# PythonOptimizers/pysparse

Hardware: AMD Instinct MI355X
Metric: CSR SpMV GB/s (7-pt Poisson, % of 8 TB/s HBM peak) + PCG iters/s (higher is better)
Workload: dtype f64

## Files before the change

### pysparse_amd/csrc/psp_csr_abi.h

```cpp

__global__ __launch_bounds__(256) void csr_validate_kernel(int nnz, int ncols, const int *__restrict__ col,
                                                           unsigned long long *bad) {
  for (long k = (long)blockIdx.x * 256 + threadIdx.x; k < nnz; k += (long)gridDim.x * 256) {
    const int c = col[k];
    if (c < 0 || c >= ncols) atomicMin(bad, (unsigned long long)k);
  }
}

extern "C" {

int psp_csr_create(int nrows, int ncols, int nnz, const int *ind_host, const int *col_host,
                   const double *val_host, psp_csr_t **out) {
  if (psp::cpu_mode()) return psp::cpu::csr_create(nrows, ncols, nnz, ind_host, col_host, val_host, out);
  if (!out || !ind_host || (nnz > 0 && (!col_host || !val_host)))
    return fail(PSP_EINVAL, "psp_csr_create: NULL argument");
  if (nrows < 0 || ncols < 0 || nnz < 0) return fail(PSP_EINVAL, "psp_csr_create: negative size");
  if (ind_host[0] != 0 || ind_host[nrows] != nnz)
    return fail(PSP_EINVAL, "psp_csr_create: ind[0] must be 0 and ind[nrows] == nnz");
  for (int i = 0; i < nrows; ++i)
    if (ind_host[i + 1] < ind_host[i])
      return fail(PSP_EINVAL, "psp_csr_create: ind not monotone at row %d", i);
  const bool check_on_device = nnz >= (1 << 22);
  if (!check_on_device)
    for (int k = 0; k < nnz; ++k)
// ... 39 lines not shown
  const long nnz = poisson_prefix(row_hi, nx, ny, nz) - poisson_prefix(row_lo, nx, ny, nz);
  if (nloc > 0x7fffffffL || nnz > 0x7fffffffL || ncols_local < 0)
    return fail(PSP_EINVAL, "psp_csr_poisson: local part exceeds 32-bit indices");
  const long reach = nz > 0 ? (long)nx * ny : nx;
  long cmin = (row_lo - reach > 0 ? row_lo - reach : 0) - col_shift;
  long cmax = (row_hi - 1 + reach < n - 1 ? row_hi - 1 + reach : n - 1) - col_shift;
  if (nloc > 0 && (cmin < 0 || cmax >= ncols_local))
    return fail(PSP_EINVAL, "psp_csr_poisson: col_shift/ncols_local do not cover the halo");
  psp_csr *A;
  PSP_TRY(alloc_csr((int)nloc, ncols_local, nnz, &A));
  int grid = (int)std::min<long>((nloc + 1 + 255) / 256, 8192);
  hipLaunchKernelGGL(poisson_csr_kernel, dim3(grid), dim3(256), 0, stream(), nx, ny, nz,
                     (long)row_lo, (long)row_hi, (long)col_shift, A->ind, A->col, A->val);
  PSP_LAUNCH_CHECK();
  PSP_TRY(finalize_csr(A));
  *out = A;
  return PSP_OK;
}

int psp_csr_poisson(int nx, int ny, int nz, psp_csr_t **out) {
  if (psp::cpu_mode()) return out ? psp::cpu::csr_poisson(nx, ny, nz, out) : fail(PSP_EINVAL, "psp_csr_poisson: NULL argument");
  const long n = (long)nx * ny * (nz > 0 ? nz : 1);
  if (n > 0x7fffffffL) return fail(PSP_EINVAL, "psp_csr_poisson: n exceeds 32-bit indices");
  return psp_csr_poisson_slab(nx, ny, nz, 0, n, 0, (int)n, out);
}

int psp_csr_poisson_big_slab(int nx, int ny, int nz, int64_t row_lo, int64_t row_hi, int64_t col_shift,
                             int ncols_local, psp_csr_t **out) {
  if (!out || nx < 2 || ny < 2 || nz < 0 || nz == 1)
    return fail(PSP_EINVAL, "psp_csr_poisson_big: grid dimensions must be >= 2 (nz = 0: 2-D)");
// ... 44 lines not shown
  hipError_t e1 = hipMalloc((void **)&ex->dia_val, sizeof(double) * nval);
  hipError_t e2 = hipMalloc((void **)&ex->dia_mask, sizeof(unsigned short) * (nblk * kDiaRows + 2));
  if (e1 != hipSuccess || e2 != hipSuccess) {
    (void)hipGetLastError();
    psp_csr_destroy(A);
    return fail(PSP_ENOMEM, "psp_csr_poisson_big: device allocation of %zu values failed", nval);
  }
  PSP_HIP(hipMemsetAsync(ex->dia_val, 0, sizeof(double) * nval, stream()));
  PSP_HIP(hipMemsetAsync(ex->dia_mask, 0, sizeof(unsigned short) * (nblk * kDiaRows + 2), stream()));
  hipLaunchKernelGGL(poisson_w4_kernel, dim3(65536), dim3(256), 0, stream(), nx, ny, nz, (long)row_lo, nloc, no,
                     ex->dia_val, ex->dia_mask);
  PSP_LAUNCH_CHECK();
  PSP_HIP(hipStreamSynchronize(stream()));
  ex->dia_no = no;
  ex->dia_state = 1;
  *out = A;
  return PSP_OK;
}

int psp_csr_poisson_big(int nx, int ny, int nz, psp_csr_t **out) {
  const long n = (long)nx * ny * (nz > 0 ? nz : 1);
  if (n > 0x7fffffffL - 256) return fail(PSP_EINVAL, "psp_csr_poisson_big: n exceeds 32-bit row indices");
  return psp_csr_poisson_big_slab(nx, ny, nz, 0, n, 0, (int)n, out);
}

int64_t psp_csr_nnz64(const psp_csr_t *A) {
  return A ? ((A->w4_only || A->nparts || A->multi) ? A->nnz64 : (int64_t)A->nnz) : 0;
}

static int create_part(int ncols, int64_t r0, int64_t r1, const int64_t *ind, const int *col, const double *val,
// ... 421 lines not shown
int psp_csr_setup_info(psp_csr_t *A, double *info4) {
  PSP_API_GUARD_H(A);
  if (!A || !info4) return fail(PSP_EINVAL, "psp_csr_setup_info: NULL argument");
  info4[0] = info4[1] = info4[2] = info4[3] = 0.0;
  if (A->host || A->multi || A->nparts) return PSP_OK;
  std::lock_guard<std::mutex> lk(g_extra_mu);
  auto it = g_extra.find(A);
  if (it == g_extra.end()) return PSP_OK;
  info4[0] = it->second.reorder_ms;
  info4[1] = (double)it->second.products;
  info4[2] = (double)reorder_after();
  info4[3] = (double)it->second.reorder_state;
  return PSP_OK;
}

int psp_csr_kernel_info(psp_csr_t *A, char *name, int name_cap, int *info) {
  PSP_API_GUARD_H(A);
  if (!A) return fail(PSP_EINVAL, "psp_csr_kernel_info: NULL handle");
  if (A->host) {
    if (name && name_cap > 0) snprintf(name, name_cap, "cpu loops (PSP_DEVICE=cpu)");
    if (info) info[0] = info[1] = info[2] = info[3] = 0;
    return PSP_OK;
  }
  if (A->multi) {
    char buf[160];
    psp::multi_describe(A->multi, buf, sizeof buf);
    if (name && name_cap > 0) snprintf(name, name_cap, "%s", buf);
    if (info) info[0] = info[1] = info[2] = info[3] = 0;
    return PSP_OK;
  }
  if (A->nparts) return psp_csr_kernel_info(A->parts[0], name, name_cap, info);
  Variant v = decode_variant(A->variant);
  if (A->w4_only) v.w4 = true;
  const char *k = "csr_spmv_stream";
  int vals[4] = {0, 0, 0, 0};
  bool w4 = false;
  if (v.w4 && A->sym_owner) {
    psp_sss *S = const_cast<psp_sss *>(A->sym_owner);
    PSP_TRY(ensure_sss_w4(S));
    if (S->w4_state == 1) {
      w4 = true;
      k = "sss_spmv_w4";
      vals[0] = S->w4_nol;
    }
  }
  if (!w4 && v.w4) {
    psp::CsrExtra *ex;
    PSP_TRY(ensure_w4(A, &ex));
    if (ex->dia_state == 1) {
      w4 = true;
      k = "csr_spmv_w4";
      vals[0] = ex->dia_no;
    }
  }
  if (!w4 && A->nrows > 0 && (v.wave || v.w1) && A->max_row_nnz <= v.tile / 2) {
    k = v.wave ? "csr_spmv_wave" : "csr_spmv_w1";
    if (v.w2) {
      ChunkTable *t;
      PSP_TRY(get_chunk_table(A, v.tile, &t));
      PSP_TRY(ensure_rowoff(A, t));
      if (t->np != 0) {
        k = "csr_spmv_w2";
        if (v.w3) {
          PSP_TRY(ensure_w3(A, t));
          vals[1] = t->max_blocks;
          {
            psp::CsrExtra *exs = nullptr;
// ... 379 lines not shown
```

### pysparse_amd/csrc/psp_csr_kernels.h

```cpp

constexpr int kBlock = 256;


__global__ void build_chunk_table(int nrows, const int *__restrict__ ind, int target, int nchunks,
                                  int2 *__restrict__ tab) {
  int c = blockIdx.x * blockDim.x + threadIdx.x;
  if (c > nchunks) return;
  int r;
  if (c == nchunks) {
    r = nrows;
  } else {
    long want = (long)c * target;
    int lo = 0, hi = nrows;
    while (lo < hi) {
      int mid = lo + ((hi - lo) >> 1);
      if ((long)ind[mid] >= want)
        hi = mid;
      else
        lo = mid + 1;
    }
    r = lo;
  }
  tab[c] = make_int2(r, ind[r]);
}
// ... 1078 lines not shown
    }
  }
}

typedef double d2u __attribute__((ext_vector_type(2), aligned(8)));

constexpr int kDiaRows = 128;
constexpr int kDiaMaxOffs = 64;
constexpr int kDiaTable = 128;
constexpr int kDiaEmpty = -0x7fffffff - 1;

struct DiaOffs {
  int o[kDiaMaxOffs];
};

__global__ void dia_offsets_kernel(int nrows, const int *__restrict__ ind, const int *__restrict__ col,
                                   int *table, int *overflow) {
  for (int r = blockIdx.x * blockDim.x + threadIdx.x; r < nrows; r += gridDim.x * blockDim.x) {
    if (*(volatile int *)overflow) return;
    int prev = -1;
    for (int k = ind[r]; k < ind[r + 1]; ++k) {
      const int c = col[k];
      if (c <= prev) {
        *overflow = 1;
        return;
      }
      prev = c;
      const int o = c - r;
      unsigned h = ((unsigned)o * 2654435761u) >> 25;
      int probes = 0;
// ... 65 lines not shown
    }
    mask[r] = (unsigned short)m;
  }
}

__global__ void dia_diag_kernel(int nrows, int no, int zero_slot, const double *__restrict__ valT,
                                const unsigned short *__restrict__ mask, double *__restrict__ diag) {
  for (long r = (long)blockIdx.x * blockDim.x + threadIdx.x; r < nrows; r += (long)gridDim.x * blockDim.x) {
    double d = 0.0;
    if (zero_slot >= 0 && ((mask[r] >> zero_slot) & 1u))
      d = valT[((size_t)(r / kDiaRows) * no + zero_slot) * kDiaRows + (size_t)(r % kDiaRows)];
    diag[r] = d;
  }
}

template <int NO, bool NTL = true, bool NTS = true>
__global__ __launch_bounds__(256) void csr_spmv_w4(
    int blk0, int blk1, int nrows, int ncols, int stripe, DiaOffs offs, const double *__restrict__ valT,
    const unsigned short *__restrict__ mask, const double *__restrict__ x, double *__restrict__ y,
    const double *__restrict__ dotv, double *__restrict__ partials, const int *__restrict__ skip,
    int use_div, double xdiv, const double *__restrict__ xdiv_dev, int dot_slot) {
  if (skip && *skip) return;
  if (xdiv_dev) xdiv = *xdiv_dev;
  __shared__ double red[4];
  const int lane = threadIdx.x & 63;
  const int wid = __builtin_amdgcn_readfirstlane(threadIdx.x >> 6);
  int vb = (int)blockIdx.x;
  if (stripe > 0) {
    const int k = vb >> 3;
    vb = ((k / stripe) * 8 + (vb & 7)) * stripe + k % stripe;
  }
  const int blk = blk0 + vb * 4 + wid;
  const long r = (long)blk * kDiaRows + 2 * lane;
  double dsum = 0.0;
  if (blk < blk1 && r < nrows) {
    const unsigned mm = *reinterpret_cast<const unsigned *>(mask + r);
    const unsigned m0 = mm & 0xffffu, m1 = mm >> 16;
    const double *vp = valT + (size_t)blk * NO * kDiaRows + 2 * lane;
    d2v v[NO];
#pragma unroll
    for (int o = 0; o < NO; ++o) v[o] = ldg<NTL>(reinterpret_cast<const d2v *>(vp + o * kDiaRows));
    d2v xv[NO];
    const long cmax = (long)ncols - 2;
    bool edge = false;
#pragma unroll
    for (int o = 0; o < NO; ++o) {
      const long c = r + offs.o[o];
      const long cc = c < 0 ? 0 : (c > cmax ? cmax : c);
      const d2u t = *reinterpret_cast<const d2u *>(x + cc);
      xv[o].x = t.x;
      xv[o].y = t.y;
      edge |= cc != c;
    }
    if (edge) {
#pragma unroll
      for (int o = 0; o < NO; ++o) {
// ... 435 lines not shown
        dsum += u.y * a1;
      }
    } else {
      y[r] = a0;
      if (dotv) dsum += dotv[r] * a0;
    }
  }
  if (partials) {
    dsum = wave_sum(dsum);
    if (lane == 0) red[wid] = dsum;
    __syncthreads();
    if (threadIdx.x == 0) partials[blockIdx.x] = red[0] + red[1] + red[2] + red[3];
  }
}

template <int NO, int PRE, bool XU = false>
__global__ __launch_bounds__(256) void csr_spmv_w4_pf(
    int nrows, int stripe, DiaOffs offs, const double *__restrict__ valT,
    const unsigned short *__restrict__ mask, const double *__restrict__ r, const double *__restrict__ dinv,
    double dc, const double *__restrict__ p_old, double *__restrict__ p_new, double *__restrict__ q,
    double beta, int first, double *__restrict__ partials, const psp::PcgDev *__restrict__ dstate,
    double *__restrict__ x = nullptr, double *__restrict__ scan_partials = nullptr) {
  double alpha_x = 0.0;
  bool xp = false;
  if (dstate) {
    if (dstate->status) return;
    beta = dstate->beta;
    first = dstate->it == 1;
    if constexpr (XU) {
      alpha_x = dstate->alpha_x;
      xp = dstate->xpend != 0;
    }
  }
  __shared__ double red[4];
  __shared__ double red2[4];
  double dmax = 0.0;
  const int lane = threadIdx.x & 63;
  const int wid = __builtin_amdgcn_readfirstlane(threadIdx.x >> 6);
  int vb = (int)blockIdx.x;
  if (stripe > 0) {
    const int k = vb >> 3;
    vb = ((k / stripe) * 8 + (vb & 7)) * stripe + k % stripe;
  }
  const int blk = vb * 4 + wid;
  const long row = (long)blk * kDiaRows + 2 * lane;
  double dsum = 0.0;
  if (row < nrows) {
    const unsigned mm = *reinterpret_cast<const unsigned *>(mask + row);
    const unsigned m0 = mm & 0xffffu, m1 = mm >> 16;
    const double *vp = valT + (size_t)blk * NO * kDiaRows + 2 * lane;
    d2v v[NO];
#pragma unroll
    for (int o = 0; o < NO; ++o) v[o] = ldg<true>(reinterpret_cast<const d2v *>(vp + o * kDiaRows));
    const long cmax = (long)nrows - 2;
    const long rc = row > cmax ? cmax : row;
    d2u rr[NO + 1], pp[NO + 1], dd[NO + 1];
    bool edge = rc != row;
#pragma unroll
    for (int o = 0; o <= NO; ++o) {
      const long c = o < NO ? row + offs.o[o] : row;
      const long cc = c < 0 ? 0 : (c > cmax ? cmax : c);
      rr[o] = *reinterpret_cast<const d2u *>(r + cc);
      if (!first) pp[o] = *reinterpret_cast<const d2u *>(p_old + cc);
      if constexpr (PRE == 1) dd[o] = *reinterpret_cast<const d2u *>(dinv + cc);
      edge |= cc != c;
    }
    if (edge) {
#pragma unroll
// ... 275 lines not shown
```

### pysparse_amd/csrc/psp_csr_select.h

```cpp
namespace psp {

static int colmask() {
#ifdef PSP_TUNING
  static const int m = [] {
    const char *e = psp::tuning_env("PSP_SPMV_COLMASK");
    return e ? atoi(e) : -1;
  }();
  return m;
#else
  return -1;
#endif
}

static int spmv_stripe() {
  static const int m = [] {
    const char *e = psp::tuning_env("PSP_SPMV_STRIPE");
    return e ? atoi(e) : -1;
  }();
  return m;
}

static int w4_auto_stripe(const psp_csr *A) {
  if (A->sym_owner) return 32;
  int plane_wgs = 0;
// ... 200 lines not shown
    PSP_TRY(ensure_sss_w4(S));
    sss = S->w4_state == 1;
  }
  if (!sss) {
    PSP_TRY(ensure_w4(A, &ex));
    if (ex->dia_state != 1 || ex->dia_no > 16) return PSP_OK;
  }
  double *pbuf = partials;
  if (partials && grid > kMaxParts) {
    PSP_TRY(ensure_big_partials(ex, grid));
    pbuf = ex->big_partials;
  }
  if (sss)
    PSP_TRY(launch_sss_w4(A->sym_owner, stripe, x, y, x, pbuf, skip, grid, 1, xdiv, xdiv_dev));
  else
    PSP_TRY(launch_w4(A, ex, stripe, 0, nblk, x, y, x, pbuf, skip, grid, 1, xdiv, xdiv_dev));
  int np = grid;
  if (pbuf != partials) {
    np = kFold;
    hipLaunchKernelGGL(fold_partials_kernel, dim3(np / 16), dim3(256), 0, stream(), pbuf, grid, partials, np);
    PSP_LAUNCH_CHECK();
  }
  if (nparts) *nparts = np;
  *available = 1;
  return PSP_OK;
}

__global__ __launch_bounds__(256) void grid_wrap_check_kernel(int n, int nx, int ny, const unsigned short *__restrict__ mask,
                                                              int *__restrict__ bad) {
  int found = 0;
  for (long r = (long)blockIdx.x * blockDim.x + threadIdx.x; r < n; r += (long)gridDim.x * blockDim.x) {
    const unsigned m = mask[r];
    const int i = (int)(r % nx), j = (int)((r / nx) % ny);
    if (((m >> 2) & 1u) && i == 0) found = 1;
    if (((m >> 4) & 1u) && i == nx - 1) found = 1;
    if (((m >> 1) & 1u) && j == 0) found = 1;
    if (((m >> 5) & 1u) && j == ny - 1) found = 1;
  }
  if (found) atomicAdd(bad, 1);
}

__global__ __launch_bounds__(256) void w4_value_range_kernel(int n, int no, const double *__restrict__ valT,
                                                             const unsigned short *__restrict__ mask, double *__restrict__ out) {
  __shared__ double smin[4][16], smax[4][16];
  double lo[16], hi[16];
  for (int o = 0; o < 16; ++o) {
    lo[o] = INFINITY;
    hi[o] = -INFINITY;
  }
  for (long r = (long)blockIdx.x * blockDim.x + threadIdx.x; r < n; r += (long)gridDim.x * blockDim.x) {
    const unsigned m = mask[r];
    const double *vp = valT + (size_t)(r / kDiaRows) * no * kDiaRows + (size_t)(r % kDiaRows);
    for (int o = 0; o < no; ++o)
      if ((m >> o) & 1u) {
        const double v = vp[(size_t)o * kDiaRows];
        lo[o] = v < lo[o] ? v : lo[o];
        hi[o] = v > hi[o] ? v : hi[o];
        if (!(v == v)) hi[o] = INFINITY, lo[o] = -INFINITY;
      }
  }
  const int lane = threadIdx.x & 63, wid = threadIdx.x >> 6;
  for (int o = 0; o < no; ++o) {
    double a = lo[o], b = hi[o];
    for (int off = 32; off > 0; off >>= 1) {
      const double a2 = __shfl_down(a, off, 64), b2 = __shfl_down(b, off, 64);
      a = a2 < a ? a2 : a;
      b = b2 > b ? b2 : b;
    }
    if (lane == 0) {
      smin[wid][o] = a;
      smax[wid][o] = b;
    }
  }
  __syncthreads();
  if ((int)threadIdx.x < no) {
    const int o = threadIdx.x;
    double a = smin[0][o], b = smax[0][o];
    for (int w = 1; w < 4; ++w) {
      a = smin[w][o] < a ? smin[w][o] : a;
      b = smax[w][o] > b ? smax[w][o] : b;
    }
    out[((size_t)blockIdx.x * no + o) * 2] = a;
    out[((size_t)blockIdx.x * no + o) * 2 + 1] = b;
  }
}

int csr_w4_view(const psp_csr *A, W4View *out, int *available) {
  *available = 0;
  Variant v = decode_variant(A->variant);
  if (A->w4_only) v.w4 = true;
  if (!v.w4 || A->nparts || A->multi || A->host || A->nrows != A->ncols || A->nrows < 2) return PSP_OK;
  psp::CsrExtra *ex;
  PSP_TRY(ensure_w4(A, &ex));
  if (ex->dia_state != 1 || ex->dia_no > 9 || !ex->dia_mask) return PSP_OK;
  out->no = ex->dia_no;
  for (int i = 0; i < 12; ++i) out->offs[i] = i < ex->dia_no ? ex->dia_offs.o[i] : 0;
  out->valT = ex->dia_val;
  out->mask = ex->dia_mask;
  out->stripe = w4_stripe(A, v);
// ... 18 lines not shown
        if (e1 != hipSuccess || e2 != hipSuccess) return fail(PSP_ENODEV, "csr_w4_view: grid check failed");
        if (hbad == 0) {
          ex->grid_state = 1;
          ex->grid_nx = s1;
          ex->grid_ny = s2 / s1;
        }
      }
    }
    if (ex->grid_state == 1) {
      out->grid3[0] = ex->grid_nx;
      out->grid3[1] = ex->grid_ny;
      out->grid3[2] = A->nrows / (ex->grid_nx * ex->grid_ny);
    }
  }
  out->constv = 0;
  if (ex->dia_no <= 12) {
    if (ex->constv_state < 0) {
      ex->constv_state = 0;
      const int no = ex->dia_no, blocks = std::min((A->nrows + 255) / 256, 512);
      double *d = nullptr;
      PSP_HIP(hipMalloc((void **)&d, sizeof(double) * 2 * no * blocks));
      hipLaunchKernelGGL(w4_value_range_kernel, dim3(blocks), dim3(256), 0, stream(), A->nrows, no, ex->dia_val, ex->dia_mask, d);
      std::vector<double> h((size_t)2 * no * blocks);
      const hipError_t e1 = hipMemcpyAsync(h.data(), d, sizeof(double) * h.size(), hipMemcpyDeviceToHost, stream());
      const hipError_t e2 = hipStreamSynchronize(stream());
      (void)hipFree(d);
      if (e1 != hipSuccess || e2 != hipSuccess) return fail(PSP_ENODEV, "csr_w4_view: value range pass failed");
      bool all = true;
      for (int o = 0; o < no && all; ++o) {
        double lo = INFINITY, hi = -INFINITY;
        for (int b = 0; b < blocks; ++b) {
          lo = std::min(lo, h[((size_t)b * no + o) * 2]);
          hi = std::max(hi, h[((size_t)b * no + o) * 2 + 1]);
        }
        if (!(lo == hi) || std::signbit(lo) != std::signbit(hi)) all = false;
        ex->constv[o] = lo;
      }
      if (all) ex->constv_state = 1;
    }
    if (ex->constv_state == 1) {
      out->constv = 1;
      for (int o = 0; o < 12; ++o) out->cval[o] = o < ex->dia_no ? ex->constv[o] : 0.0;
    }
  }
  *available = 1;
  return PSP_OK;
}

int csr_spmv_pfx_launch(const psp_csr *A, const double *r, const double *dinv, const double *p_old, double *p_new,
                        double *q, double *x, double *partials, int *nparts, const PcgDev *dstate, int *available) {
  *available = 0;
  Variant v = decode_variant(A->variant);
  if (!v.w4 || A->nparts || A->sym_owner || A->nrows != A->ncols || A->nrows < 2 || !dstate || !partials) return PSP_OK;
  psp::CsrExtra *ex;
  PSP_TRY(ensure_w4(A, &ex));
  if (ex->dia_state != 1 || ex->dia_no > 8) return PSP_OK;
  const int stripe = w4_stripe(A, v);
  const int nblk = (A->nrows + kDiaRows - 1) / kDiaRows;
  const int grid = w4_grid(nblk, stripe);
  if (grid > kMaxParts) return PSP_OK;
  double dc = 0.0;
  const int pre = !dinv ? 0 : (dinv_constant(dinv, A->nrows, &dc) ? 2 : 1);
  double *scan = partials + 2 * (size_t)kMaxParts;
#define PSP_PFX(NO, PRE)                                                                                    \
  hipLaunchKernelGGL((csr_spmv_w4_pf<NO, PRE, true>), dim3(grid), dim3(256), 0, stream(), A->nrows, stripe, \
                     ex->dia_offs, ex->dia_val, ex->dia_mask, r, dinv, dc, p_old, p_new, q, 0.0, 0, partials, dstate, x, scan)
#define PSP_PFX_NO(NO)                \
  case NO:                            \
    if (pre == 0) PSP_PFX(NO, 0);     \
    else if (pre == 1) PSP_PFX(NO, 1); \
    else PSP_PFX(NO, 2);              \
    break
  switch (ex->dia_no) {
    PSP_PFX_NO(1); PSP_PFX_NO(2); PSP_PFX_NO(3); PSP_PFX_NO(4); PSP_PFX_NO(5); PSP_PFX_NO(6); PSP_PFX_NO(7); PSP_PFX_NO(8);
    default:
      return PSP_OK;
  }
#undef PSP_PFX_NO
#undef PSP_PFX
  PSP_LAUNCH_CHECK();
  *nparts = grid;
  *available = 1;
  return PSP_OK;
}

bool csr_spmv_has_skip(const psp_csr *A) {
// ... 45 lines not shown
  if (t->np == 0) return PSP_OK;
  psp::setup_mark("first use: chunk table + row offsets");
  PSP_TRY(ensure_w3(A, t));
  psp::setup_mark("first use: w3 tables on the stored numbering");
  psp::CsrExtra *exs = nullptr;
  int mode = 0;
  PSP_TRY(pick_scattered(A, t, &exs, &mode));
  if (mode != 1) return PSP_OK;
  exs->reordered->variant = A->variant;
  *R = exs->reordered;
  *perm = exs->perm;
  *inv = exs->inv;
  return PSP_OK;
}

int csr_spmv_launch(const psp_csr *A, const double *x, double *y, const double *dotv,
                    double *partials, int *nparts, const int *skip) {
  Workspace *w;
  PSP_TRY(workspace(&w));
  psp::setup_mark(nullptr);
  if (A->nparts) {
    double *tmp = w->partials + (size_t)(kSlots - 1) * kMaxParts;
    if (partials && (partials == tmp || (long)A->nparts * kFold > kMaxParts))
      return fail(PSP_EINVAL, "csr_spmv_launch: partitioned matrix needs a partial-sum slot other than the last");
    for (int p = 0; p < A->nparts; ++p) {
      const psp_csr *P = A->parts[p];
      if (P->nrows == 0) continue;
      const int r0 = A->part_row0[p];
      int np = 0;
      PSP_TRY(csr_spmv_launch(P, x, y + r0, (partials && dotv) ? dotv + r0 : nullptr, partials ? tmp : nullptr, &np,
                              skip));
      if (partials) {
        hipLaunchKernelGGL(fold_partials_kernel, dim3(kFold / 16), dim3(256), 0, stream(), tmp, np,
                           partials + (size_t)p * kFold, kFold);
        PSP_LAUNCH_CHECK();
      }
    }
    if (nparts) *nparts = A->nparts * kFold;
    return PSP_OK;
  }
  Variant v = decode_variant(A->variant);
  if (A->w4_only) v.w4 = true;
  if (v.w4 && A->sym_owner) {
    psp_sss *S = const_cast<psp_sss *>(A->sym_owner);
    PSP_TRY(ensure_sss_w4(S));
    if (S->w4_state == 1) {
// ... 22 lines not shown
      return PSP_OK;
    }
  }
  if (v.w4) {
    psp::CsrExtra *ex;
    PSP_TRY(ensure_w4(A, &ex));
    if (ex->dia_state == 1) {
      const int stripe = w4_stripe(A, v);
      const int nblk = (A->nrows + kDiaRows - 1) / kDiaRows;
      const int grid = w4_grid(nblk, stripe);
      double *pbuf = partials;
      if (partials && grid > kMaxParts) {
        PSP_TRY(ensure_big_partials(ex, grid));
        pbuf = ex->big_partials;
      }
      PSP_TRY(launch_w4(A, ex, stripe, 0, nblk, x, y, dotv, pbuf, skip, grid));
      int np = grid;
      if (pbuf != partials) {
        np = kFold;
        hipLaunchKernelGGL(fold_partials_kernel, dim3(np / 16), dim3(256), 0, stream(), pbuf, grid,
                           partials, np);
        PSP_LAUNCH_CHECK();
      }
      if (nparts) *nparts = np;
      return PSP_OK;
    }
  }
  if (A->w4_only) return fail(PSP_EINVAL, "this operator exists only in the w4 layout (psp_csr_poisson_big)");
  if ((v.wave || v.w1) && A->max_row_nnz > v.tile / 2) {
    v.wave = v.w1 = v.w2 = false;
    v.tile = 2048;
// ... 277 lines not shown
    PSP_TRY(ensure_w4(A, &ex));
    if (ex->dia_state == 1) {
      const int nblk = (A->nrows + kDiaRows - 1) / kDiaRows;
      int ba = (row_a + kDiaRows - 1) / kDiaRows, bb = row_b / kDiaRows;
      if (row_b >= A->nrows) bb = nblk;
      if (bb < ba) bb = ba;
      const int stripe = w4_stripe(A, v);
      const int g1 = bb > ba ? w4_grid(bb - ba, stripe) : 0;
      const int g2 = ba > 0 ? w4_grid(ba, stripe) : 0;
      const int g3 = nblk > bb ? w4_grid(nblk - bb, stripe) : 0;
      double *pbuf = nullptr;
      if (partials) {
        PSP_TRY(ensure_big_partials(ex, g1 + g2 + g3 + 8));
        pbuf = ex->big_partials;
      }
      if (g1) PSP_TRY(launch_w4(A, ex, stripe, ba, bb, x, y, dotv, pbuf, skip, g1));
      if (wait && wait(ctx)) return fail(PSP_ECALLBACK, "halo wait callback failed");
      if (g2) PSP_TRY(launch_w4(A, ex, stripe, 0, ba, x, y, dotv, pbuf ? pbuf + g1 : nullptr, skip, g2));
      if (g3) PSP_TRY(launch_w4(A, ex, stripe, bb, nblk, x, y, dotv, pbuf ? pbuf + g1 + g2 : nullptr, skip, g3));
      if (partials) {
        hipLaunchKernelGGL(fold_partials_kernel, dim3(kFold / 16), dim3(256), 0, stream(), pbuf, g1 + g2 + g3,
                           partials, kFold);
        PSP_LAUNCH_CHECK();
        if (nparts) *nparts = kFold;
      }
      return PSP_OK;
    }
  }
  ChunkTable *t = nullptr;
  bool ok = v.w2 && A->max_row_nnz <= v.tile / 2 && row_a < row_b;
  if (ok) {
    PSP_TRY(get_chunk_table(const_cast<psp_csr *>(A), v.tile, &t));
    PSP_TRY(ensure_rowoff(A, t));
    ok = t->np != 0;
// ... 188 lines not shown
    if (hipStreamSynchronize(s_dn) != hipSuccess) err = 1;
  });
  const int stripe = w4_stripe(A, v);
  int rc = PSP_OK;
  for (int k = 0; k < K && rc == PSP_OK && !err; ++k) {
    const long r0 = k * kPipeChunk, r1 = std::min(n, r0 + kPipeChunk);
    const long xhi = std::min(n, r1 + omax + 2);
    const int need = (int)((xhi + kPipeChunk - 1) / kPipeChunk);
    while (up_done.load(std::memory_order_acquire) < need && !err) std::this_thread::yield();
    if (err) break;
    if (hipStreamWaitEvent(stream(), ev_up[need - 1], 0) != hipSuccess) {
      err = 1;
      break;
    }
    const int b0 = (int)(r0 / kDiaRows), b1 = (int)((r1 + kDiaRows - 1) / kDiaRows);
    rc = launch_w4(A, ex, stripe, b0, b1, xd, yd, nullptr, nullptr, nullptr, w4_grid(b1 - b0, stripe));
    if (rc == PSP_OK && hipEventRecord(ev_k[k], stream()) != hipSuccess) err = 1;
    k_done.store(k + 1, std::memory_order_release);
  }
  if (rc != PSP_OK || err) err = 1;
  k_done.store(K, std::memory_order_release);
  uploader.join();
  downloader.join();
  (void)hipStreamSynchronize(stream());
  for (int k = 0; k < K; ++k) {
    (void)hipEventDestroy(ev_up[k]);
    (void)hipEventDestroy(ev_k[k]);
  }
  if (rc != PSP_OK) return rc;
  if (err) return fail(PSP_ENODEV, "host-pointer matvec pipeline: %s", hipGetErrorString(hipGetLastError()));
  *done = true;
// ... 34 lines not shown
```

### pysparse_amd/csrc/psp_csr_tables.h

```cpp

struct ChunkTable {
  int tile = 0;
  int target = 0;
  int nchunks = 0;
  int2 *tab = nullptr;
  int max_rows = -1;
  int np = 0;
  unsigned short *rowoff = nullptr;
  int nb = -1;
  int max_blocks = 0;
  int outliers = 0;
  int *blist = nullptr;
  unsigned short *col16 = nullptr;
  int nb6 = -1;
  int direct6 = 0;
  int *blist6 = nullptr;
  int nu = -1;
  int max_cols = 0;
  int *ulist = nullptr;
  unsigned short *colu = nullptr;
  int sched_state = -1;
  int sched_grid = 0;
  int *perm = nullptr;
  int half_band = 0;
// ... 358 lines not shown
  const int per = (nwg + 7) / 8;
  const int grid = per * 8;
  std::vector<int> perm((size_t)grid, -1);
  for (int j = 0; j < 8; ++j)
    for (int p = 0; p < per; ++p) {
      const long src = (long)j * per + p;
      if (src < nwg) perm[(size_t)p * 8 + j] = keys[(size_t)src].wg;
    }
  PSP_HIP(hipMalloc((void **)&t->perm, sizeof(int) * (size_t)grid));
  PSP_HIP(hipMemcpy(t->perm, perm.data(), sizeof(int) * (size_t)grid, hipMemcpyHostToDevice));
  t->sched_grid = grid;
  t->sched_state = 1;
  return PSP_OK;
}

static int ensure_w4(const psp_csr *A, psp::CsrExtra **out) {
  std::lock_guard<std::mutex> lk(g_extra_mu);
  psp::CsrExtra &ex = g_extra[A];
  *out = &ex;
  if (ex.dia_state >= 0) return PSP_OK;
  ex.dia_state = 0;
  static const bool off = [] {
    const char *e = psp::tuning_env("PSP_SPMV_W4");
    return e && atoi(e) == 0;
  }();
  if (off || A->nrows < 1 || A->ncols < 2 || A->nnz < 1 || A->max_row_nnz > kDiaMaxOffs) return PSP_OK;
  ScratchDev tab_mem;
  PSP_HIP(hipMalloc(&tab_mem.p, (kDiaTable + 1) * sizeof(int)));
  int *d_tab = (int *)tab_mem.p;
  int init[kDiaTable + 1];
// ... 51 lines not shown
    hipLaunchKernelGGL(dia_build_kernel<unsigned long long>, dim3(bgrid), dim3(256), 0, stream(), A->nrows, no,
                       ex.dia_offs, A->ind, A->col, A->val, ex.dia_val, ex.dia_mask64);
  } else if (m32) {
    PSP_HIP(hipMemsetAsync(ex.dia_mask32, 0, sizeof(unsigned) * nmask, stream()));
    hipLaunchKernelGGL(dia_build_kernel<unsigned>, dim3(bgrid), dim3(256), 0, stream(), A->nrows, no, ex.dia_offs,
                       A->ind, A->col, A->val, ex.dia_val, ex.dia_mask32);
  } else {
    PSP_HIP(hipMemsetAsync(ex.dia_mask, 0, sizeof(unsigned short) * nmask, stream()));
    hipLaunchKernelGGL(dia_build_kernel<unsigned short>, dim3(bgrid), dim3(256), 0, stream(), A->nrows, no,
                       ex.dia_offs, A->ind, A->col, A->val, ex.dia_val, ex.dia_mask);
  }
  PSP_LAUNCH_CHECK();
  PSP_HIP(hipStreamSynchronize(stream()));
  ex.dia_no = no;
  ex.dia_state = 1;
  return PSP_OK;
}

static bool w4_dot_reload() {
  const char *e = psp::tuning_env("PSP_W4_DOT_RELOAD");
  return e && atoi(e) != 0;
}

static int launch_w4(const psp_csr *A, const psp::CsrExtra *ex, int stripe, int b0, int b1, const double *x,
                     double *y, const double *dotv, double *pbuf, const int *skip, int grid, int use_div = 0,
                     double xdiv = 1.0, const double *xdiv_dev = nullptr) {
  if (use_div && ex->dia_no > 16) return fail(PSP_EINVAL, "csr_spmv_w4x has no scaled form");
  const int flags = (A->variant >= 0 ? A->variant : 0) >> 23 & 3;
  int dot_slot = -1;
  if (dotv && ex->dia_no <= 16 && !w4_dot_reload()) {
    const intptr_t diff = (intptr_t)dotv - (intptr_t)x;
    if (diff % (intptr_t)sizeof(double) == 0)
      for (int k = 0; k < ex->dia_no; ++k)
        if ((intptr_t)ex->dia_offs.o[k] == diff / (intptr_t)sizeof(double)) dot_slot = k;
  }
#define PSP_W4_F(NO, NTL, NTS)                                                                       \
  hipLaunchKernelGGL((csr_spmv_w4<NO, NTL, NTS>), dim3(grid), dim3(256), 0, stream(), b0, b1, A->nrows, \
                     A->ncols, stripe, ex->dia_offs, ex->dia_val, ex->dia_mask, x, y, dotv, pbuf, skip,  \
                     use_div, xdiv, xdiv_dev, dot_slot)
#define PSP_W4(NO)                                                                                   \
  case NO:                                                                                           \
    if (flags == 0) PSP_W4_F(NO, true, true);                                                        \
    else if (flags == 1) PSP_W4_F(NO, false, true);                                                  \
    else if (flags == 2) PSP_W4_F(NO, true, false);                                                  \
    else PSP_W4_F(NO, false, false);                                                                 \
    break
  switch (ex->dia_no) {
    PSP_W4(1); PSP_W4(2); PSP_W4(3); PSP_W4(4); PSP_W4(5); PSP_W4(6); PSP_W4(7); PSP_W4(8);
    PSP_W4(9); PSP_W4(10); PSP_W4(11); PSP_W4(12); PSP_W4(13); PSP_W4(14); PSP_W4(15); PSP_W4(16);
#define PSP_W4X(NO)                                                                                  \
  case NO:                                                                                           \
    hipLaunchKernelGGL((csr_spmv_w4x<NO>), dim3(grid), dim3(256), 0, stream(), b0, b1, A->nrows,      \
                       A->ncols, stripe, ex->dia_offs, ex->dia_val, ex->dia_mask32, x, y, dotv, pbuf, \
                       skip);                                                                        \
    break
    PSP_W4X(17); PSP_W4X(18); PSP_W4X(19); PSP_W4X(20); PSP_W4X(21); PSP_W4X(22); PSP_W4X(23); PSP_W4X(24);
    PSP_W4X(25); PSP_W4X(26); PSP_W4X(27); PSP_W4X(28); PSP_W4X(29); PSP_W4X(30); PSP_W4X(31); PSP_W4X(32);
#undef PSP_W4X
    default:
      if (ex->dia_no > 32 && ex->dia_no <= kDiaMaxOffs && ex->dia_mask64) {
        hipLaunchKernelGGL(csr_spmv_w4y, dim3(grid), dim3(256), 0, stream(), b0, b1, A->nrows, A->ncols, stripe,
                           ex->dia_no, ex->dia_offs_dev, ex->dia_val, ex->dia_mask64, x, y, dotv, pbuf, skip);
        break;
      }
      return fail(PSP_EINVAL, "csr_spmv_w4: %d offsets", ex->dia_no);
  }
#undef PSP_W4
#undef PSP_W4_F
  PSP_LAUNCH_CHECK();
  return PSP_OK;
}

static int w4_grid(int nblocks, int stripe) {
  int grid = (nblocks + 3) / 4;
  if (stripe > 0) grid = (grid + 8 * stripe - 1) / (8 * stripe) * (8 * stripe);
  return grid;
}

static int ensure_big_partials(psp::CsrExtra *ex, int cap) {
  std::lock_guard<std::mutex> lk(g_extra_mu);
  if (ex->big_cap < cap) {
    if (ex->big_partials) (void)hipFree(ex->big_partials);
// ... 419 lines not shown
```

Baseline: 6139.

## Specialize W4 SpMV and PCG kernels for constant-valued diagonals

At setup, a device pass computes per-diagonal min/max of stored values using an order-preserving integer encoding. When every diagonal is constant, the values are passed to the SpMV and fused PCG kernels as arguments instead of being streamed from memory. This removes the value-array traffic for stencil matrices such as the Poisson operator. In exchange it adds a setup pass with a host sync and more template instantiations, and it applies only to large unpartitioned matrices.

After: 4388. 28.5% lower.

```diff
diff --git a/pysparse_amd/csrc/psp_csr_abi.h b/pysparse_amd/csrc/psp_csr_abi.h
--- a/pysparse_amd/csrc/psp_csr_abi.h
+++ b/pysparse_amd/csrc/psp_csr_abi.h
@@ -77,6 +77,10 @@
                      (long)row_lo, (long)row_hi, (long)col_shift, A->ind, A->col, A->val);
   PSP_LAUNCH_CHECK();
   PSP_TRY(finalize_csr(A));
+  if (row_lo != 0 || row_hi != n) {
+    std::lock_guard<std::mutex> lk(g_extra_mu);
+    g_extra[A].constv_state = 0;
+  }
   *out = A;
   return PSP_OK;
 }
@@ -151,6 +155,14 @@
   PSP_HIP(hipStreamSynchronize(stream()));
   ex->dia_no = no;
   ex->dia_state = 1;
+  ex->constv_state = 0;
+  if (row_lo == 0 && row_hi == n) {
+    const int rc = w4_constv_pass(A->nrows, ex);
+    if (rc != PSP_OK) {
+      psp_csr_destroy(A);
+      return rc;
+    }
+  }
   *out = A;
   return PSP_OK;
 }
@@ -602,7 +614,13 @@
   return PSP_OK;
 }
 
+static int kernel_info_impl(psp_csr_t *A, char *name, int name_cap, int *info, bool part);
+
 int psp_csr_kernel_info(psp_csr_t *A, char *name, int name_cap, int *info) {
+  return kernel_info_impl(A, name, name_cap, info, false);
+}
+
+static int kernel_info_impl(psp_csr_t *A, char *name, int name_cap, int *info, bool part) {
   PSP_API_GUARD_H(A);
   if (!A) return fail(PSP_EINVAL, "psp_csr_kernel_info: NULL handle");
   if (A->host) {
@@ -617,7 +635,7 @@
     if (info) info[0] = info[1] = info[2] = info[3] = 0;
     return PSP_OK;
   }
-  if (A->nparts) return psp_csr_kernel_info(A->parts[0], name, name_cap, info);
+  if (A->nparts) return kernel_info_impl(A->parts[0], name, name_cap, info, true);
   Variant v = decode_variant(A->variant);
   if (A->w4_only) v.w4 = true;
   const char *k = "csr_spmv_stream";
@@ -638,7 +656,7 @@
     if (ex->dia_state == 1) {
       w4 = true;
       k = "csr_spmv_w4";
-      vals[0] = ex->dia_no;
+      vals[0] = (!part && w4_cv(A, ex)) ? 0 : ex->dia_no;
     }
   }
   if (!w4 && A->nrows > 0 && (v.wave || v.w1) && A->max_row_nnz <= v.tile / 2) {
diff --git a/pysparse_amd/csrc/psp_csr_kernels.h b/pysparse_amd/csrc/psp_csr_kernels.h
--- a/pysparse_amd/csrc/psp_csr_kernels.h
+++ b/pysparse_amd/csrc/psp_csr_kernels.h
@@ -1116,6 +1116,11 @@
   int o[kDiaMaxOffs];
 };
 
+constexpr int kDiaCvOffs = 16;
+struct DiaVals {
+  double v[kDiaCvOffs];
+};
+
 __global__ void dia_offsets_kernel(int nrows, const int *__restrict__ ind, const int *__restrict__ col,
                                    int *table, int *overflow) {
   for (int r = blockIdx.x * blockDim.x + threadIdx.x; r < nrows; r += gridDim.x * blockDim.x) {
@@ -1211,12 +1216,61 @@
   }
 }
 
-template <int NO, bool NTL = true, bool NTS = true>
+__global__ __launch_bounds__(256) void w4_value_range_kernel(int n, int no, const double *__restrict__ valT,
+                                                             const unsigned short *__restrict__ mask,
+                                                             unsigned long long *__restrict__ out) {
+  __shared__ unsigned long long smin[4][kDiaCvOffs], smax[4][kDiaCvOffs];
+  unsigned long long lo[kDiaCvOffs], hi[kDiaCvOffs];
+  for (int o = 0; o < kDiaCvOffs; ++o) {
+    lo[o] = ~0ull;
+    hi[o] = 0ull;
+  }
+  for (long r = (long)blockIdx.x * blockDim.x + threadIdx.x; r < n; r += (long)gridDim.x * blockDim.x) {
+    const unsigned m = mask[r];
+    const double *vp = valT + (size_t)(r / kDiaRows) * no * kDiaRows + (size_t)(r % kDiaRows);
+#pragma unroll
+    for (int o = 0; o < kDiaCvOffs; ++o)
+      if (o < no && ((m >> o) & 1u)) {
+        const double v = vp[(size_t)o * kDiaRows];
+        const unsigned long long b = (unsigned long long)__double_as_longlong(v);
+        const unsigned long long k = b ^ ((b >> 63) ? ~0ull : (1ull << 63));
+        lo[o] = (v == v) ? (k < lo[o] ? k : lo[o]) : 0ull;
+        hi[o] = (v == v) ? (k > hi[o] ? k : hi[o]) : ~0ull;
+      }
+  }
+  const int lane = threadIdx.x & 63, wid = threadIdx.x >> 6;
+#pragma unroll
+  for (int o = 0; o < kDiaCvOffs; ++o) {
+    unsigned long long a = lo[o], b = hi[o];
+    for (int off = 32; off > 0; off >>= 1) {
+      const unsigned long long a2 = __shfl_down(a, off, 64), b2 = __shfl_down(b, off, 64);
+      a = a2 < a ? a2 : a;
+      b = b2 > b ? b2 : b;
+    }
+    if (lane == 0) {
+      smin[wid][o] = a;
+      smax[wid][o] = b;
+    }
+  }
+  __syncthreads();
+  if ((int)threadIdx.x < no) {
+    const int o = threadIdx.x;
+    unsigned long long a = smin[0][o], b = smax[0][o];
+    for (int w = 1; w < 4; ++w) {
+      a = smin[w][o] < a ? smin[w][o] : a;
+      b = smax[w][o] > b ? smax[w][o] : b;
+    }
+    out[((size_t)blockIdx.x * no + o) * 2] = a;
+    out[((size_t)blockIdx.x * no + o) * 2 + 1] = b;
+  }
+}
+
+template <int NO, bool NTL = true, bool NTS = true, bool CV = false>
 __global__ __launch_bounds__(256) void csr_spmv_w4(
     int blk0, int blk1, int nrows, int ncols, int stripe, DiaOffs offs, const double *__restrict__ valT,
     const unsigned short *__restrict__ mask, const double *__restrict__ x, double *__restrict__ y,
     const double *__restrict__ dotv, double *__restrict__ partials, const int *__restrict__ skip,
-    int use_div, double xdiv, const double *__restrict__ xdiv_dev, int dot_slot) {
+    int use_div, double xdiv, const double *__restrict__ xdiv_dev, int dot_slot, DiaVals cv = DiaVals()) {
   if (skip && *skip) return;
   if (xdiv_dev) xdiv = *xdiv_dev;
   __shared__ double red[4];
@@ -1233,10 +1287,15 @@
   if (blk < blk1 && r < nrows) {
     const unsigned mm = *reinterpret_cast<const unsigned *>(mask + r);
     const unsigned m0 = mm & 0xffffu, m1 = mm >> 16;
-    const double *vp = valT + (size_t)blk * NO * kDiaRows + 2 * lane;
     d2v v[NO];
-#pragma unroll
-    for (int o = 0; o < NO; ++o) v[o] = ldg<NTL>(reinterpret_cast<const d2v *>(vp + o * kDiaRows));
+    if constexpr (CV) {
+#pragma unroll
+      for (int o = 0; o < NO; ++o) v[o].x = v[o].y = cv.v[o];
+    } else {
+      const double *vp = valT + (size_t)blk * NO * kDiaRows + 2 * lane;
+#pragma unroll
+      for (int o = 0; o < NO; ++o) v[o] = ldg<NTL>(reinterpret_cast<const d2v *>(vp + o * kDiaRows));
+    }
     d2v xv[NO];
     const long cmax = (long)ncols - 2;
     bool edge = false;
@@ -1702,13 +1761,13 @@
   }
 }
 
-template <int NO, int PRE, bool XU = false>
+template <int NO, int PRE, bool XU = false, bool CV = false>
 __global__ __launch_bounds__(256) void csr_spmv_w4_pf(
     int nrows, int stripe, DiaOffs offs, const double *__restrict__ valT,
     const unsigned short *__restrict__ mask, const double *__restrict__ r, const double *__restrict__ dinv,
     double dc, const double *__restrict__ p_old, double *__restrict__ p_new, double *__restrict__ q,
     double beta, int first, double *__restrict__ partials, const psp::PcgDev *__restrict__ dstate,
-    double *__restrict__ x = nullptr, double *__restrict__ scan_partials = nullptr) {
+    double *__restrict__ x = nullptr, double *__restrict__ scan_partials = nullptr, DiaVals cv = DiaVals()) {
   double alpha_x = 0.0;
   bool xp = false;
   if (dstate) {
@@ -1736,10 +1795,15 @@
   if (row < nrows) {
     const unsigned mm = *reinterpret_cast<const unsigned *>(mask + row);
     const unsigned m0 = mm & 0xffffu, m1 = mm >> 16;
-    const double *vp = valT + (size_t)blk * NO * kDiaRows + 2 * lane;
     d2v v[NO];
-#pragma unroll
-    for (int o = 0; o < NO; ++o) v[o] = ldg<true>(reinterpret_cast<const d2v *>(vp + o * kDiaRows));
+    if constexpr (CV) {
+#pragma unroll
+      for (int o = 0; o < NO; ++o) v[o].x = v[o].y = cv.v[o];
+    } else {
+      const double *vp = valT + (size_t)blk * NO * kDiaRows + 2 * lane;
+#pragma unroll
+      for (int o = 0; o < NO; ++o) v[o] = ldg<true>(reinterpret_cast<const d2v *>(vp + o * kDiaRows));
+    }
     const long cmax = (long)nrows - 2;
     const long rc = row > cmax ? cmax : row;
     d2u rr[NO + 1], pp[NO + 1], dd[NO + 1];
diff --git a/pysparse_amd/csrc/psp_csr_select.h b/pysparse_amd/csrc/psp_csr_select.h
--- a/pysparse_amd/csrc/psp_csr_select.h
+++ b/pysparse_amd/csrc/psp_csr_select.h
@@ -238,7 +238,7 @@
   if (sss)
     PSP_TRY(launch_sss_w4(A->sym_owner, stripe, x, y, x, pbuf, skip, grid, 1, xdiv, xdiv_dev));
   else
-    PSP_TRY(launch_w4(A, ex, stripe, 0, nblk, x, y, x, pbuf, skip, grid, 1, xdiv, xdiv_dev));
+    PSP_TRY(launch_w4(A, ex, stripe, 0, nblk, x, y, x, pbuf, skip, grid, true, 1, xdiv, xdiv_dev));
   int np = grid;
   if (pbuf != partials) {
     np = kFold;
@@ -262,51 +262,6 @@
     if (((m >> 5) & 1u) && j == ny - 1) found = 1;
   }
   if (found) atomicAdd(bad, 1);
-}
-
-__global__ __launch_bounds__(256) void w4_value_range_kernel(int n, int no, const double *__restrict__ valT,
-                                                             const unsigned short *__restrict__ mask, double *__restrict__ out) {
-  __shared__ double smin[4][16], smax[4][16];
-  double lo[16], hi[16];
-  for (int o = 0; o < 16; ++o) {
-    lo[o] = INFINITY;
-    hi[o] = -INFINITY;
-  }
-  for (long r = (long)blockIdx.x * blockDim.x + threadIdx.x; r < n; r += (long)gridDim.x * blockDim.x) {
-    const unsigned m = mask[r];
-    const double *vp = valT + (size_t)(r / kDiaRows) * no * kDiaRows + (size_t)(r % kDiaRows);
-    for (int o = 0; o < no; ++o)
-      if ((m >> o) & 1u) {
-        const double v = vp[(size_t)o * kDiaRows];
-        lo[o] = v < lo[o] ? v : lo[o];
-        hi[o] = v > hi[o] ? v : hi[o];
-        if (!(v == v)) hi[o] = INFINITY, lo[o] = -INFINITY;
-      }
-  }
-  const int lane = threadIdx.x & 63, wid = threadIdx.x >> 6;
-  for (int o = 0; o < no; ++o) {
-    double a = lo[o], b = hi[o];
-    for (int off = 32; off > 0; off >>= 1) {
-      const double a2 = __shfl_down(a, off, 64), b2 = __shfl_down(b, off, 64);
-      a = a2 < a ? a2 : a;
-      b = b2 > b ? b2 : b;
-    }
-    if (lane == 0) {
-      smin[wid][o] = a;
-      smax[wid][o] = b;
-    }
-  }
-  __syncthreads();
-  if ((int)threadIdx.x < no) {
-    const int o = threadIdx.x;
-    double a = smin[0][o], b = smax[0][o];
-    for (int w = 1; w < 4; ++w) {
-      a = smin[w][o] < a ? smin[w][o] : a;
-      b = smax[w][o] > b ? smax[w][o] : b;
-    }
-    out[((size_t)blockIdx.x * no + o) * 2] = a;
-    out[((size_t)blockIdx.x * no + o) * 2 + 1] = b;
-  }
 }
 
 int csr_w4_view(const psp_csr *A, W4View *out, int *available) {
@@ -355,34 +310,9 @@
     }
   }
   out->constv = 0;
-  if (ex->dia_no <= 12) {
-    if (ex->constv_state < 0) {
-      ex->constv_state = 0;
-      const int no = ex->dia_no, blocks = std::min((A->nrows + 255) / 256, 512);
-      double *d = nullptr;
-      PSP_HIP(hipMalloc((void **)&d, sizeof(double) * 2 * no * blocks));
-      hipLaunchKernelGGL(w4_value_range_kernel, dim3(blocks), dim3(256), 0, stream(), A->nrows, no, ex->dia_val, ex->dia_mask, d);
-      std::vector<double> h((size_t)2 * no * blocks);
-      const hipError_t e1 = hipMemcpyAsync(h.data(), d, sizeof(double) * h.size(), hipMemcpyDeviceToHost, stream());
-      const hipError_t e2 = hipStreamSynchronize(stream());
-      (void)hipFree(d);
-      if (e1 != hipSuccess || e2 != hipSuccess) return fail(PSP_ENODEV, "csr_w4_view: value range pass failed");
-      bool all = true;
-      for (int o = 0; o < no && all; ++o) {
-        double lo = INFINITY, hi = -INFINITY;
-        for (int b = 0; b < blocks; ++b) {
-          lo = std::min(lo, h[((size_t)b * no + o) * 2]);
-          hi = std::max(hi, h[((size_t)b * no + o) * 2 + 1]);
-        }
-        if (!(lo == hi) || std::signbit(lo) != std::signbit(hi)) all = false;
-        ex->constv[o] = lo;
-      }
-      if (all) ex->constv_state = 1;
-    }
-    if (ex->constv_state == 1) {
-      out->constv = 1;
-      for (int o = 0; o < 12; ++o) out->cval[o] = o < ex->dia_no ? ex->constv[o] : 0.0;
-    }
+  if (ex->dia_no <= 12 && ex->constv_state == 1) {
+    out->constv = 1;
+    for (int o = 0; o < 12; ++o) out->cval[o] = o < ex->dia_no ? ex->constv[o] : 0.0;
   }
   *available = 1;
   return PSP_OK;
@@ -403,14 +333,18 @@
   double dc = 0.0;
   const int pre = !dinv ? 0 : (dinv_constant(dinv, A->nrows, &dc) ? 2 : 1);
   double *scan = partials + 2 * (size_t)kMaxParts;
-#define PSP_PFX(NO, PRE)                                                                                    \
-  hipLaunchKernelGGL((csr_spmv_w4_pf<NO, PRE, true>), dim3(grid), dim3(256), 0, stream(), A->nrows, stripe, \
-                     ex->dia_offs, ex->dia_val, ex->dia_mask, r, dinv, dc, p_old, p_new, q, 0.0, 0, partials, dstate, x, scan)
-#define PSP_PFX_NO(NO)                \
-  case NO:                            \
-    if (pre == 0) PSP_PFX(NO, 0);     \
-    else if (pre == 1) PSP_PFX(NO, 1); \
-    else PSP_PFX(NO, 2);              \
+  const bool cv = w4_cv(A, ex);
+  DiaVals vals;
+  for (int o = 0; o < kDiaCvOffs; ++o) vals.v[o] = cv ? ex->constv[o] : 0.0;
+#define PSP_PFX(NO, PRE, CV)                                                                                    \
+  hipLaunchKernelGGL((csr_spmv_w4_pf<NO, PRE, true, CV>), dim3(grid), dim3(256), 0, stream(), A->nrows, stripe, \
+                     ex->dia_offs, ex->dia_val, ex->dia_mask, r, dinv, dc, p_old, p_new, q, 0.0, 0, partials, dstate, x, \
+                     scan, vals)
+#define PSP_PFX_NO(NO)                                                              \
+  case NO:                                                                          \
+    if (pre == 0) { if (cv) PSP_PFX(NO, 0, true); else PSP_PFX(NO, 0, false); }      \
+    else if (pre == 1) { if (cv) PSP_PFX(NO, 1, true); else PSP_PFX(NO, 1, false); } \
+    else { if (cv) PSP_PFX(NO, 2, true); else PSP_PFX(NO, 2, false); }               \
     break
   switch (ex->dia_no) {
     PSP_PFX_NO(1); PSP_PFX_NO(2); PSP_PFX_NO(3); PSP_PFX_NO(4); PSP_PFX_NO(5); PSP_PFX_NO(6); PSP_PFX_NO(7); PSP_PFX_NO(8);
@@ -486,8 +420,16 @@
   return PSP_OK;
 }
 
+static int spmv_launch_impl(const psp_csr *A, const double *x, double *y, const double *dotv, double *partials,
+                            int *nparts, const int *skip, bool allow_cv);
+
 int csr_spmv_launch(const psp_csr *A, const double *x, double *y, const double *dotv,
                     double *partials, int *nparts, const int *skip) {
+  return spmv_launch_impl(A, x, y, dotv, partials, nparts, skip, true);
+}
+
+static int spmv_launch_impl(const psp_csr *A, const double *x, double *y, const double *dotv, double *partials,
+                            int *nparts, const int *skip, bool allow_cv) {
   Workspace *w;
   PSP_TRY(workspace(&w));
   psp::setup_mark(nullptr);
@@ -500,8 +442,8 @@
       if (P->nrows == 0) continue;
       const int r0 = A->part_row0[p];
       int np = 0;
-      PSP_TRY(csr_spmv_launch(P, x, y + r0, (partials && dotv) ? dotv + r0 : nullptr, partials ? tmp : nullptr, &np,
-                              skip));
+      PSP_TRY(spmv_launch_impl(P, x, y + r0, (partials && dotv) ? dotv + r0 : nullptr, partials ? tmp : nullptr, &np,
+                               skip, false));
       if (partials) {
         hipLaunchKernelGGL(fold_partials_kernel, dim3(kFold / 16), dim3(256), 0, stream(), tmp, np,
                            partials + (size_t)p * kFold, kFold);
@@ -554,7 +496,7 @@
         PSP_TRY(ensure_big_partials(ex, grid));
         pbuf = ex->big_partials;
       }
-      PSP_TRY(launch_w4(A, ex, stripe, 0, nblk, x, y, dotv, pbuf, skip, grid));
+      PSP_TRY(launch_w4(A, ex, stripe, 0, nblk, x, y, dotv, pbuf, skip, grid, allow_cv));
       int np = grid;
       if (pbuf != partials) {
         np = kFold;
@@ -862,10 +804,10 @@
         PSP_TRY(ensure_big_partials(ex, g1 + g2 + g3 + 8));
         pbuf = ex->big_partials;
       }
-      if (g1) PSP_TRY(launch_w4(A, ex, stripe, ba, bb, x, y, dotv, pbuf, skip, g1));
+      if (g1) PSP_TRY(launch_w4(A, ex, stripe, ba, bb, x, y, dotv, pbuf, skip, g1, false));
       if (wait && wait(ctx)) return fail(PSP_ECALLBACK, "halo wait callback failed");
-      if (g2) PSP_TRY(launch_w4(A, ex, stripe, 0, ba, x, y, dotv, pbuf ? pbuf + g1 : nullptr, skip, g2));
-      if (g3) PSP_TRY(launch_w4(A, ex, stripe, bb, nblk, x, y, dotv, pbuf ? pbuf + g1 + g2 : nullptr, skip, g3));
+      if (g2) PSP_TRY(launch_w4(A, ex, stripe, 0, ba, x, y, dotv, pbuf ? pbuf + g1 : nullptr, skip, g2, false));
+      if (g3) PSP_TRY(launch_w4(A, ex, stripe, bb, nblk, x, y, dotv, pbuf ? pbuf + g1 + g2 : nullptr, skip, g3, false));
       if (partials) {
         hipLaunchKernelGGL(fold_partials_kernel, dim3(kFold / 16), dim3(256), 0, stream(), pbuf, g1 + g2 + g3,
                            partials, kFold);
@@ -1084,7 +1026,7 @@
       break;
     }
     const int b0 = (int)(r0 / kDiaRows), b1 = (int)((r1 + kDiaRows - 1) / kDiaRows);
-    rc = launch_w4(A, ex, stripe, b0, b1, xd, yd, nullptr, nullptr, nullptr, w4_grid(b1 - b0, stripe));
+    rc = launch_w4(A, ex, stripe, b0, b1, xd, yd, nullptr, nullptr, nullptr, w4_grid(b1 - b0, stripe), true);
     if (rc == PSP_OK && hipEventRecord(ev_k[k], stream()) != hipSuccess) err = 1;
     k_done.store(k + 1, std::memory_order_release);
   }
diff --git a/pysparse_amd/csrc/psp_csr_tables.h b/pysparse_amd/csrc/psp_csr_tables.h
--- a/pysparse_amd/csrc/psp_csr_tables.h
+++ b/pysparse_amd/csrc/psp_csr_tables.h
@@ -396,6 +396,46 @@
   return PSP_OK;
 }
 
+static int w4_constv_pass(int nrows, psp::CsrExtra *ex) {
+  ex->constv_state = 0;
+  if (ex->dia_no < 1 || ex->dia_no > kDiaCvOffs || !ex->dia_mask || nrows < 1) return PSP_OK;
+  const int no = ex->dia_no, blocks = std::min((nrows + 255) / 256, 2048);
+  ScratchDev mem;
+  PSP_HIP(hipMalloc(&mem.p, sizeof(unsigned long long) * 2 * no * blocks));
+  hipLaunchKernelGGL(w4_value_range_kernel, dim3(blocks), dim3(256), 0, stream(), nrows, no, ex->dia_val, ex->dia_mask,
+                     (unsigned long long *)mem.p);
+  PSP_LAUNCH_CHECK();
+  std::vector<unsigned long long> h((size_t)2 * no * blocks);
+  PSP_HIP(hipMemcpyAsync(h.data(), mem.p, sizeof(unsigned long long) * h.size(), hipMemcpyDeviceToHost, stream()));
+  PSP_HIP(hipStreamSynchronize(stream()));
+  for (int o = 0; o < no; ++o) {
+    unsigned long long lo = ~0ull, hi = 0ull;
+    for (int b = 0; b < blocks; ++b) {
+      lo = std::min(lo, h[((size_t)b * no + o) * 2]);
+      hi = std::max(hi, h[((size_t)b * no + o) * 2 + 1]);
+    }
+    if (lo != hi) return PSP_OK;
+    const unsigned long long bits = lo ^ ((lo >> 63) ? (1ull << 63) : ~0ull);
+    memcpy(&ex->constv[o], &bits, sizeof(double));
+  }
+  ex->constv_state = 1;
+  return PSP_OK;
+}
+
+static int w4_cv_mode() {
+  const char *e = psp::tuning_env("PSP_W4_CV");
+  return e ? atoi(e) : 1;
+}
+
+constexpr int kW4CvMinRows = 1 << 21;
+
+static bool w4_cv(const psp_csr *A, const psp::CsrExtra *ex) {
+  if (ex->dia_state != 1 || ex->constv_state != 1 || ex->dia_no > kDiaCvOffs || A->nparts || A->multi || A->sym_owner)
+    return false;
+  const int mode = w4_cv_mode();
+  return mode == 2 || (mode == 1 && A->nrows >= kW4CvMinRows);
+}
+
 static int ensure_w4(const psp_csr *A, psp::CsrExtra **out) {
   std::lock_guard<std::mutex> lk(g_extra_mu);
   psp::CsrExtra &ex = g_extra[A];
@@ -477,7 +517,7 @@
   PSP_HIP(hipStreamSynchronize(stream()));
   ex.dia_no = no;
   ex.dia_state = 1;
-  return PSP_OK;
+  return ex.constv_state < 0 ? w4_constv_pass(A->nrows, &ex) : PSP_OK;
 }
 
 static bool w4_dot_reload() {
@@ -486,10 +526,13 @@
 }
 
 static int launch_w4(const psp_csr *A, const psp::CsrExtra *ex, int stripe, int b0, int b1, const double *x,
-                     double *y, const double *dotv, double *pbuf, const int *skip, int grid, int use_div = 0,
+                     double *y, const double *dotv, double *pbuf, const int *skip, int grid, bool cv, int use_div = 0,
                      double xdiv = 1.0, const double *xdiv_dev = nullptr) {
   if (use_div && ex->dia_no > 16) return fail(PSP_EINVAL, "csr_spmv_w4x has no scaled form");
   const int flags = (A->variant >= 0 ? A->variant : 0) >> 23 & 3;
+  cv = cv && w4_cv(A, ex);
+  DiaVals vals;
+  for (int o = 0; o < kDiaCvOffs; ++o) vals.v[o] = cv ? ex->constv[o] : 0.0;
   int dot_slot = -1;
   if (dotv && ex->dia_no <= 16 && !w4_dot_reload()) {
     const intptr_t diff = (intptr_t)dotv - (intptr_t)x;
@@ -501,9 +544,15 @@
   hipLaunchKernelGGL((csr_spmv_w4<NO, NTL, NTS>), dim3(grid), dim3(256), 0, stream(), b0, b1, A->nrows, \
                      A->ncols, stripe, ex->dia_offs, ex->dia_val, ex->dia_mask, x, y, dotv, pbuf, skip,  \
                      use_div, xdiv, xdiv_dev, dot_slot)
+#define PSP_W4_CV(NO, NTS)                                                                                  \
+  hipLaunchKernelGGL((csr_spmv_w4<NO, true, NTS, true>), dim3(grid), dim3(256), 0, stream(), b0, b1, A->nrows, \
+                     A->ncols, stripe, ex->dia_offs, ex->dia_val, ex->dia_mask, x, y, dotv, pbuf, skip,         \
+                     use_div, xdiv, xdiv_dev, dot_slot, vals)
 #define PSP_W4(NO)                                                                                   \
   case NO:                                                                                           \
-    if (flags == 0) PSP_W4_F(NO, true, true);                                                        \
+    if (cv && (flags & 2) == 0) PSP_W4_CV(NO, true);                                                 \
+    else if (cv) PSP_W4_CV(NO, false);                                                               \
+    else if (flags == 0) PSP_W4_F(NO, true, true);                                                   \
     else if (flags == 1) PSP_W4_F(NO, false, true);                                                  \
     else if (flags == 2) PSP_W4_F(NO, true, false);                                                  \
     else PSP_W4_F(NO, false, false);                                                                 \
@@ -529,6 +578,7 @@
       return fail(PSP_EINVAL, "csr_spmv_w4: %d offsets", ex->dia_no);
   }
 #undef PSP_W4
+#undef PSP_W4_CV
 #undef PSP_W4_F
   PSP_LAUNCH_CHECK();
   return PSP_OK;
```
